# StellaOrg/ImplicitBVH.jl

Measured on AMD Instinct MI355X. Metric: BVH build+traverse throughput, higher is better.
Workload: dtype f32; 1 GPU; 1000000 random BSphere{Float32} leaves per GPU, BBox{Float32} nodes, UInt32 Morton, Int32 index, build + LVT self-traverse + read of the contact count (BASELINE.json configs[1]); leaves_per_gpu=1000000, leaves_total=1000000, contacts_total=1763579, parallelism=single GPU

## Files before the change

implicitbvh.jl_amd/csrc/ibvh_build.hip:

```cpp
#include "ibvh_common.hpp"
#include "ibvh_radix.hpp"
#include "ibvh_msd.hpp"

namespace ibvh {
namespace rsort {
struct FirstPassPlan {
    int tpb, ipt, num_tiles;
    uint32_t *tile_hist;
    uint32_t mask;
    int shift, bits;
};
FirstPassPlan first_pass_plan(int64_t n, int key_bits, int key_bytes, void *scratch);
bool uses_hybrid(int64_t n, int key_bits, int key_bytes);
int sort_pairs(int key_bytes, int key_bits, int64_t n, void *keys, void *vals, void *keys_alt, void *vals_alt,
               bool vals_implicit, int32_t *result_in_alt, void *scratch, size_t scratch_sz, hipStream_t st,
               bool first_hist_done, const RecordArgs *records);
size_t scratch_bytes(int64_t n);
}

namespace build {

constexpr int EXT_TPB = 256;
constexpr int EXT_MAX_BLOCKS = 2048;
constexpr int EXT_FOLD_BLOCKS = 512;

template <class T> IBVH_D T wave_min(T v) {
#pragma unroll
    for (int o = 32; o > 0; o >>= 1) {
        T t = __shfl_xor(v, o, 64);
        v = v < t ? v : t;
    }
    return v;
}
template <class T> IBVH_D T wave_max(T v) {
#pragma unroll
    for (int o = 32; o > 0; o >>= 1) {
        T t = __shfl_xor(v, o, 64);
        v = v > t ? v : t;
    }
    return v;
}

template <class V>
__global__ __launch_bounds__(EXT_TPB) void extrema_partial_kernel(const char *__restrict__ recs, int64_t stride, int64_t n,
                                                                  typename V::elt *__restrict__ partials) {
    using T = typename V::elt;
    T mn[3] = {float_max<T>(), float_max<T>(), float_max<T>()};
    T mx[3] = {float_min_normal<T>(), float_min_normal<T>(), float_min_normal<T>()};
    for (int64_t i = (int64_t)blockIdx.x * EXT_TPB + threadIdx.x; i < n; i += (int64_t)gridDim.x * EXT_TPB) {
        V v = load_vol<V>(recs + i * stride);
        T c[3];
        center(v, c);
#pragma unroll
        for (int k = 0; k < 3; ++k) {
            mn[k] = mn[k] < c[k] ? mn[k] : c[k];
            mx[k] = mx[k] > c[k] ? mx[k] : c[k];
        }
    }
    __shared__ T s[EXT_TPB / 64][6];
    const int lane = threadIdx.x & 63, w = threadIdx.x >> 6;
#pragma unroll
    for (int k = 0; k < 3; ++k) {
        T a = wave_min(mn[k]), b = wave_max(mx[k]);
        if (lane == 0) {
            s[w][k] = a;
            s[w][3 + k] = b;
        }
    }
    __syncthreads();
    if (threadIdx.x < 6) {
        T v = s[0][threadIdx.x];
        for (int i = 1; i < EXT_TPB / 64; ++i) {
            T t = s[i][threadIdx.x];
            v = threadIdx.x < 3 ? (v < t ? v : t) : (v > t ? v : t);
        }
        partials[(int64_t)blockIdx.x * 6 + threadIdx.x] = v;
    }
}

struct SkipsOut {
    TreeDev tree;
    void *skips;
    int index_bytes;
};
IBVH_D void write_skips(const SkipsOut &so) {
    const int64_t level = (int64_t)threadIdx.x + 1;
    if (so.skips == nullptr || level > so.tree.levels) return;
    const int64_t v = level_skips(so.tree.levels, so.tree.virtual_leaves, level);
    if (so.index_bytes == 4) ((int32_t *)so.skips)[level - 1] = (int32_t)v;
    else ((int64_t *)so.skips)[level - 1] = v;
}

template <class T>
__global__ __launch_bounds__(EXT_TPB) void extrema_final_kernel(const T *__restrict__ partials, int nparts, int expand,
                                                                T *__restrict__ out, T *__restrict__ out2, SkipsOut so) {
    write_skips(so);
    T mn[3] = {float_max<T>(), float_max<T>(), float_max<T>()};
    T mx[3] = {float_min_normal<T>(), float_min_normal<T>(), float_min_normal<T>()};
    for (int i = threadIdx.x; i < nparts; i += EXT_TPB) {
#pragma unroll
        for (int k = 0; k < 3; ++k) {
            T a = partials[i * 6 + k], b = partials[i * 6 + 3 + k];
            mn[k] = mn[k] < a ? mn[k] : a;
            mx[k] = mx[k] > b ? mx[k] : b;
        }
    }
    __shared__ T s[EXT_TPB / 64][6];
    const int lane = threadIdx.x & 63, w = threadIdx.x >> 6;
#pragma unroll
    for (int k = 0; k < 3; ++k) {
        T a = wave_min(mn[k]), b = wave_max(mx[k]);
        if (lane == 0) {
            s[w][k] = a;
            s[w][3 + k] = b;
        }
    }
    __syncthreads();
    if (threadIdx.x < 6) {
        T v = s[0][threadIdx.x];
        for (int i = 1; i < EXT_TPB / 64; ++i) {
            T t = s[i][threadIdx.x];
            v = threadIdx.x < 3 ? (v < t ? v : t) : (v > t ? v : t);
        }
        if (expand) {
            const T rp = relative_precision<T>(), fm = float_min_normal<T>();
            T a = rp * ibvh_abs(v);
            v = threadIdx.x < 3 ? (v - a) - fm : (v + a) + fm;
        }
        out[threadIdx.x] = v;
        if (out2) out2[threadIdx.x] = v;
    }
}

template <class T> __global__ void extrema_set_kernel(T *out, T *out2, double a0, double a1, double a2, double b0, double b1, double b2, SkipsOut so) {
    write_skips(so);
    if (threadIdx.x == 0) {
        out[0] = T(a0);
        out[1] = T(a1);
        out[2] = T(a2);
        out[3] = T(b0);
        out[4] = T(b1);
        out[5] = T(b2);
        if (out2)
            for (int k = 0; k < 6; ++k) out2[k] = out[k];
    }
}

template <class V, class K>
__global__ __launch_bounds__(256) void encode_kernel(const char *__restrict__ recs, int64_t stride, int64_t n,
                                                     const typename V::elt *__restrict__ ext, int morton_type,
                                                     K *__restrict__ keys) {
    using T = typename V::elt;
    const T mins[3] = {ext[0], ext[1], ext[2]}, maxs[3] = {ext[3], ext[4], ext[5]};
    for (int64_t i = (int64_t)blockIdx.x * 256 + threadIdx.x; i < n; i += (int64_t)gridDim.x * 256) {
        V v = load_vol<V>(recs + i * stride);
        T c[3];
        center(v, c);
        keys[i] = (K)morton_encode_single(c, mins, maxs, morton_type);
    }
}

template <class T> struct ExtremaFold {
    const T *partials;
    int nparts;
    T *out, *out2;
    SkipsOut so;
};
template <class V, class K>
// ... 24 lines not shown
        for (int k = 0; k < 3; ++k) {
            const T a = wave_min(mn[k]), b = wave_max(mx[k]);
            if (lane == 0) {
                s_fold[w][k] = a;
                s_fold[w][3 + k] = b;
            }
        }
        __syncthreads();
        if (threadIdx.x < 6) {
            T v = s_fold[0][threadIdx.x];
            for (int i = 1; i < (int)(blockDim.x >> 6); ++i) {
                const T t = s_fold[i][threadIdx.x];
                v = threadIdx.x < 3 ? (v < t ? v : t) : (v > t ? v : t);
            }
            const T rp = relative_precision<T>(), fm = float_min_normal<T>();
            const T a = rp * ibvh_abs(v);
            v = threadIdx.x < 3 ? (v - a) - fm : (v + a) + fm;
            s_ext[threadIdx.x] = v;
            if (blockIdx.x == 0) {
                fold.out[threadIdx.x] = v;
                if (fold.out2) fold.out2[threadIdx.x] = v;
            }
        }
    }
    __syncthreads();
    const T *bounds = fold.partials != nullptr ? s_ext : ext;
    const T mins[3] = {bounds[0], bounds[1], bounds[2]}, maxs[3] = {bounds[3], bounds[4], bounds[5]};
    const int64_t base = (int64_t)blockIdx.x * tile_elems;
    for (int j = threadIdx.x; j < tile_elems; j += blockDim.x) {
        const int64_t i = base + j;
        if (i < n) {
            V v = load_vol<V>(recs + i * stride);
            T c[3];
            center(v, c);
            const K k = (K)morton_encode_single(c, mins, maxs, morton_type);
            keys[i] = k;
            atomicAdd(&h[(uint32_t)(k >> shift) & mask], 1u);
        }
    }
    __syncthreads();
    if (tile_major)
        for (int d = threadIdx.x; d <= (int)mask; d += blockDim.x) tile_hist[(int64_t)blockIdx.x * (mask + 1) + d] = h[d];
    else
        for (int d = threadIdx.x; d <= (int)mask; d += blockDim.x) tile_hist[(int64_t)d * num_tiles + blockIdx.x] = h[d];
}

template <class V, class I, class K>
__global__ __launch_bounds__(256) void gather_kernel(const char *__restrict__ src, int64_t src_stride, int src_wrapped,
                                                     LeafLayout lay, const K *__restrict__ keys,
                                                     const uint32_t *__restrict__ perm, int64_t n, char *__restrict__ dst) {
    extern __shared__ __attribute__((aligned(16))) unsigned char g_smem[];
    const int lane = threadIdx.x & 63, wv = threadIdx.x >> 6;
    const int words = lay.stride >> 3;
    uint64_t *stage = (uint64_t *)g_smem + (size_t)wv * 64 * words;
    const int64_t nchunks = ceil_div_dev(n, 256);
    for (int64_t c = blockIdx.x; c < nchunks; c += gridDim.x) {
        const int64_t i = c * 256 + threadIdx.x;
        const int64_t wave_first = c * 256 + wv * 64;
        if (i < n) {
            const uint32_t p = perm[i];
            const char *s = src + (int64_t)p * src_stride;
            V v;
            if (sizeof(V) % 16 == 0 && (src_stride & 15) == 0) v = load_vol16<V>(s);
            else v = load_vol<V>(s);
            I idx = src_wrapped ? load_index<I>(s, lay) : (I)((int64_t)p + 1);
            char *d = (char *)(stage + (size_t)lane * words);
            store_vol(d, v);
            *(I *)(d + lay.index_off) = idx;
            store_morton(d, lay, (uint64_t)keys[i]);
        }
        __builtin_amdgcn_wave_barrier();
        const int64_t wave_n = n - wave_first < 64 ? n - wave_first : 64;
        if (wave_n > 0) {
            uint64_t *out = (uint64_t *)(dst + wave_first * lay.stride);
            const int total = (int)wave_n * words;
            for (int g = lane; g < total; g += 64) out[g] = stage[g];
        }
        __builtin_amdgcn_wave_barrier();
    }
}

constexpr int AGG_TPB = 256;
constexpr int CH_LEVELS = 9;

template <class N>
IBVH_D void fold_up(N *s_nodes, N mine, int64_t level, int64_t nreal, const TreeDev &tree, int64_t built_level, N *__restrict__ nodes) {
    const int t = threadIdx.x;
    int count = AGG_TPB;
#pragma unroll 1
    for (int s = 1; s < CH_LEVELS; ++s) {
        if (level - 1 < built_level) break;
        __syncthreads();
        if (t < count) s_nodes[t] = mine;
        __syncthreads();
        count >>= 1;
        level -= 1;
        const int64_t child_real = nreal;
        nreal = level_num_real(tree.levels, tree.virtual_leaves, level);
        const int64_t i = (int64_t)blockIdx.x * count + t;
        if ((t < count) && (i < nreal)) {
            N a = s_nodes[2 * t];
            if (2 * i + 1 < child_real) mine = merge_to(a, s_nodes[2 * t + 1], (N *)nullptr);
            else mine = a;
            nodes[level_start(tree.levels, tree.virtual_leaves, level) - 1 + i] = mine;
        }
    }
}

template <class L, class N, bool FROM_LEAVES>
__global__ __launch_bounds__(AGG_TPB) void aggregate_kernel(const char *__restrict__ in, int64_t in_stride, int64_t in_level,
                                                            TreeDev tree, int64_t built_level, N *__restrict__ nodes) {
    __shared__ N s_nodes[AGG_TPB];
    const int t = threadIdx.x;
    int64_t level = in_level - 1;
    const int64_t in_real = FROM_LEAVES ? tree.real_leaves : level_num_real(tree.levels, tree.virtual_leaves, in_level);
    const int64_t i = (int64_t)blockIdx.x * AGG_TPB + t;
    const int64_t nreal = level_num_real(tree.levels, tree.virtual_leaves, level);
    N mine;
    if (i < nreal) {
        int64_t l = 2 * i, r = 2 * i + 1;
        if constexpr (FROM_LEAVES) {
            L a = load_vol<L>(in + l * in_stride);
            if (r < in_real) {
                L b = load_vol<L>(in + r * in_stride);
                mine = merge_to(a, b, (N *)nullptr);
            } else {
                mine = convert_to(a, (N *)nullptr);
            }
        } else {
            N a = load_vol<N>(in + l * in_stride);
            if (r < in_real) {
                N b = load_vol<N>(in + r * in_stride);
                mine = merge_to(a, b, (N *)nullptr);
            } else {
                mine = a;
            }
        }
        nodes[level_start(tree.levels, tree.virtual_leaves, level) - 1 + i] = mine;
    }
    fold_up<N>(s_nodes, mine, level, nreal, tree, built_level, nodes);
}

template <class L, class N, class I>
__global__ __launch_bounds__(AGG_TPB) void refit_kernel(char *__restrict__ leaves, LeafLayout lay, const char *__restrict__ volumes,
                                                        int64_t m, uint32_t *flag, TreeDev tree, int64_t built_level,
                                                        N *__restrict__ nodes) {
    __shared__ N s_nodes[AGG_TPB];
    const int64_t i = (int64_t)blockIdx.x * AGG_TPB + threadIdx.x;
    const bool one_leaf = tree.levels == 1;
    const int64_t level = tree.levels - 1;
    const int64_t nreal = one_leaf ? 1 : level_num_real(tree.levels, tree.virtual_leaves, level);
    N mine;
    if (i < nreal) {
        const bool has_b = !one_leaf && 2 * i + 1 < tree.real_leaves;
        char *ra = leaves + 2 * i * lay.stride, *rb = ra + lay.stride;
        const I ia = load_index<I>(ra, lay), ib = has_b ? load_index<I>(rb, lay) : I(1);
        const bool oka = ia >= 1 && (int64_t)ia <= m, okb = ib >= 1 && (int64_t)ib <= m;
        const char *sa = oka ? volumes + ((int64_t)ia - 1) * (int64_t)sizeof(L) : ra;
        const char *sb = okb ? volumes + ((int64_t)ib - 1) * (int64_t)sizeof(L) : rb;
        L a, b;
        if constexpr (sizeof(L) % 16 == 0) {
            a = oka && ((uintptr_t)volumes & 15) == 0 ? load_vol16<L>(sa) : load_vol<L>(sa);
            if (has_b) b = okb && ((uintptr_t)volumes & 15) == 0 ? load_vol16<L>(sb) : load_vol<L>(sb);
        } else {
            a = load_vol<L>(sa);
            if (has_b) b = load_vol<L>(sb);
        }
        if (oka) store_vol(ra, a);
        if (has_b && okb) store_vol(rb, b);
        if (flag && !(oka && okb)) *flag = 1u;
        if (one_leaf) return;
        mine = has_b ? merge_to(a, b, (N *)nullptr) : convert_to(a, (N *)nullptr);
        nodes[level_start(tree.levels, tree.virtual_leaves, level) - 1 + i] = mine;
    }
    if (one_leaf) return;
    fold_up<N>(s_nodes, mine, level, nreal, tree, built_level, nodes);
}

constexpr int AGG_TOP_TPB = 1024, AGG_TOP_MAX = 4096, AGG_TOP_LDS_BYTES = 128 * 1024;
template <class N, bool IN_LDS>
__global__ __launch_bounds__(AGG_TOP_TPB) void aggregate_top_kernel(TreeDev tree, int64_t in_level, int64_t built_level, N *nodes) {
    if constexpr (IN_LDS) {
        extern __shared__ __attribute__((aligned(16))) unsigned char top_smem[];
        N *s = (N *)top_smem;
        int64_t have = level_num_real(tree.levels, tree.virtual_leaves, in_level);
        {
            const N *in = nodes + (level_start(tree.levels, tree.virtual_leaves, in_level) - 1);
            for (int64_t i = threadIdx.x; i < have; i += AGG_TOP_TPB) s[i] = load_vol<N>(in + i);
        }
        __syncthreads();
        for (int64_t level = in_level - 1; level >= built_level && level >= 1; --level) {
            const int64_t nreal = level_num_real(tree.levels, tree.virtual_leaves, level);
            N *out = nodes + (level_start(tree.levels, tree.virtual_leaves, level) - 1);
            N mine[2];
#pragma unroll
            for (int k = 0; k < 2; ++k) {
                const int64_t i = threadIdx.x + (int64_t)k * AGG_TOP_TPB;
                if (i < nreal) mine[k] = (2 * i + 1 < have) ? merge_to(s[2 * i], s[2 * i + 1], (N *)nullptr) : s[2 * i];
            }
            __syncthreads();
#pragma unroll
            for (int k = 0; k < 2; ++k) {
                const int64_t i = threadIdx.x + (int64_t)k * AGG_TOP_TPB;
                if (i < nreal) {
                    s[i] = mine[k];
                    store_vol(out + i, mine[k]);
                }
            }
            __syncthreads();
            have = nreal;
        }
        return;
    }
    for (int64_t level = in_level - 1; level >= built_level && level >= 1; --level) {
        const int64_t nreal = level_num_real(tree.levels, tree.virtual_leaves, level);
        const int64_t child_real = level_num_real(tree.levels, tree.virtual_leaves, level + 1);
        const N *in = nodes + (level_start(tree.levels, tree.virtual_leaves, level + 1) - 1);
        N *out = nodes + (level_start(tree.levels, tree.virtual_leaves, level) - 1);
        for (int64_t i = threadIdx.x; i < nreal; i += AGG_TOP_TPB) {
            const N a = load_vol<N>(in + 2 * i);
            if (2 * i + 1 < child_real) store_vol(out + i, merge_to(a, load_vol<N>(in + 2 * i + 1), (N *)nullptr));
            else store_vol(out + i, a);
        }
        __threadfence_block();
        __syncthreads();
    }
}

struct RefitGather {
    LeafLayout lay;
    int index_type;
    const void *volumes;
    int64_t m;
    uint32_t *flag;
};

template <class L, class N>
int aggregate(const char *leaves, int64_t leaf_stride, const ibvh_tree &tree, int64_t built_level, N *nodes, hipStream_t st,
              const RefitGather *gather = nullptr) {
    if (tree.real_nodes < 2 && !gather) return IBVH_OK;
    TreeDev td{tree.levels, tree.real_leaves, tree.virtual_leaves};
    int64_t in_level = tree.levels;
    {
        int64_t nreal = tree.levels > 1 ? level_num_real(tree.levels, tree.virtual_leaves, in_level - 1) : 1;
        int64_t eff_built = built_level > tree.levels - 1 ? tree.levels - 1 : built_level;
        if (gather) {
            int e = dispatch_index(gather->index_type, [&](auto it) -> int {
                using I = typename decltype(it)::type;
                IBVH_LAUNCH((refit_kernel<L, N, I>), dim3((unsigned)ceil_div(nreal, AGG_TPB)), dim3(AGG_TPB), 0, st,
                            (char *)leaves, gather->lay, (const char *)gather->volumes, gather->m, gather->flag, td, eff_built, nodes);
                return IBVH_OK;
            });
            if (e) return e;
        } else {
            IBVH_LAUNCH((aggregate_kernel<L, N, true>), dim3((unsigned)ceil_div(nreal, AGG_TPB)), dim3(AGG_TPB), 0, st,
                               leaves, leaf_stride, in_level, td, eff_built, nodes);
        }
        IBVH_LAUNCH_CHECK();
        if (tree.real_nodes < 2) return IBVH_OK;
        in_level = in_level - CH_LEVELS;
    }
    while (in_level - 1 >= built_level && in_level - 1 >= 1) {
        if (level_num_real(tree.levels, tree.virtual_leaves, in_level) <= AGG_TOP_MAX) {
            const size_t top_bytes = (size_t)level_num_real(tree.levels, tree.virtual_leaves, in_level) * sizeof(N);
            if (top_bytes <= (size_t)AGG_TOP_LDS_BYTES) {
                IBVH_HIP_CHECK(hipFuncSetAttribute((const void *)aggregate_top_kernel<N, true>, hipFuncAttributeMaxDynamicSharedMemorySize, AGG_TOP_LDS_BYTES));
                IBVH_LAUNCH((aggregate_top_kernel<N, true>), dim3(1), dim3(AGG_TOP_TPB), top_bytes, st, td, in_level, built_level, nodes);
            } else {
                IBVH_LAUNCH((aggregate_top_kernel<N, false>), dim3(1), dim3(AGG_TOP_TPB), 0, st, td, in_level, built_level, nodes);
            }
            IBVH_LAUNCH_CHECK();
            break;
        }
        int64_t nreal = level_num_real(tree.levels, tree.virtual_leaves, in_level - 1);
        const char *in = (const char *)(nodes + (level_start(tree.levels, tree.virtual_leaves, in_level) - 1));
        IBVH_LAUNCH((aggregate_kernel<L, N, false>), dim3((unsigned)ceil_div(nreal, AGG_TPB)), dim3(AGG_TPB), 0, st,
                           in, (int64_t)sizeof(N), in_level, td, built_level, nodes);
        IBVH_LAUNCH_CHECK();
        in_level -= CH_LEVELS;
    }
    return IBVH_OK;
}

template <class I> __global__ void skips_kernel(TreeDev tree, I *skips) {
    int64_t level = threadIdx.x + 1;
    if (level <= tree.levels) skips[level - 1] = (I)level_skips(tree.levels, tree.virtual_leaves, level);
}

inline int grid_for(int64_t n, int tpb, int max_blocks) {
    int64_t b = ceil_div(n, tpb);
    return (int)(b < 1 ? 1 : (b > max_blocks ? max_blocks : b));
}

struct Scratch {
    char *partials;
    char *extrema;
    char *keys, *keys_alt;
    char *vals, *vals_alt;
    char *records;
    char *records2;
    char *sort;
    size_t total;
};
inline int morton_key_bits(int morton_type);
inline Scratch carve(char *base, int64_t n, int key_bytes, int64_t leaf_bytes, int morton_type) {
    Scratch s;
    size_t off = 0;
    auto take = [&](size_t bytes) {
        char *p = base ? base + off : nullptr;
        off += (size_t)align_up((int64_t)bytes, 256);
        return p;
    };
    s.partials = take((size_t)EXT_MAX_BLOCKS * 6 * 8);
    s.extrema = take(64);
    s.keys = take((size_t)n * key_bytes);
    s.keys_alt = take((size_t)n * key_bytes);
    s.vals = take((size_t)n * 4);
    s.vals_alt = take((size_t)n * 4);
    s.records = take((size_t)n * leaf_bytes);
    s.records2 = take((size_t)n * leaf_bytes);
    const size_t a = rsort::scratch_bytes(n), b = msd::scratch_bytes(n, morton_key_bits(morton_type), key_bytes, (int)leaf_bytes);
    s.sort = take(a > b ? a : b);
    s.total = off;
    return s;
}

template <class V> int extrema_partials(const char *recs, int64_t stride, int64_t n, char *partials, hipStream_t st, int *nparts) {
    using T = typename V::elt;
    const int blocks = grid_for(n, EXT_TPB * 4, EXT_FOLD_BLOCKS);
    IBVH_LAUNCH((extrema_partial_kernel<V>), dim3(blocks), dim3(EXT_TPB), 0, st, recs, stride, n, (T *)partials);
    *nparts = blocks;
    return IBVH_OK;
}
template <class V>
int extrema(const char *recs, int64_t stride, int64_t n, int expand, typename V::elt *out, char *partials, hipStream_t st,
            typename V::elt *out2 = nullptr, SkipsOut so = SkipsOut{TreeDev{0, 0, 0}, nullptr, 4}) {
    using T = typename V::elt;
    int blocks = grid_for(n, EXT_TPB * 4, EXT_MAX_BLOCKS);
    IBVH_LAUNCH((extrema_partial_kernel<V>), dim3(blocks), dim3(EXT_TPB), 0, st, recs, stride, n, (T *)partials);
    IBVH_LAUNCH((extrema_final_kernel<T>), dim3(1), dim3(EXT_TPB), 0, st, (const T *)partials, blocks, expand, out, out2, so);
    IBVH_LAUNCH_CHECK();
    return IBVH_OK;
}

template <class V>
int encode(const char *recs, int64_t stride, int64_t n, const typename V::elt *ext, int morton_type, void *keys, hipStream_t st) {
    int blocks = grid_for(n, 256, 256 * 16);
    if (morton_type == IBVH_U64)
        IBVH_LAUNCH((encode_kernel<V, uint64_t>), dim3(blocks), dim3(256), 0, st, recs, stride, n, ext, morton_type,
                           (uint64_t *)keys);
    else
        IBVH_LAUNCH((encode_kernel<V, uint32_t>), dim3(blocks), dim3(256), 0, st, recs, stride, n, ext, morton_type,
                           (uint32_t *)keys);
    IBVH_LAUNCH_CHECK();
    return IBVH_OK;
}

inline int morton_key_bits(int morton_type) { return morton_type == IBVH_U16 ? 15 : (morton_type == IBVH_U32 ? 30 : 63); }

}
}

using namespace ibvh;
using namespace ibvh::build;

extern "C" {

ibvh_status ibvh_build_scratch_bytes(const ibvh_types *types, int64_t n, size_t *bytes_out) {
    if (!types || !bytes_out) return IBVH_ERR_INVALID_ARG;
    ibvh_layout lay;
    if (!layout_of(*types, lay)) return IBVH_ERR_UNSUPPORTED;
    if (n < 1) return IBVH_ERR_DOMAIN;
    int kb = types->morton_type == IBVH_U64 ? 8 : 4;
    *bytes_out = carve(nullptr, n, kb, lay.leaf_bytes, types->morton_type).total;
    return IBVH_OK;
}

ibvh_status ibvh_extrema(const ibvh_types *types, const void *records, int32_t wrapped, int64_t n, int32_t expand,
                         void *extrema_out, void *scratch, size_t scratch_bytes, void *stream) {
    if (!types || !records || !extrema_out || !scratch) return IBVH_ERR_INVALID_ARG;
    if (n < 1) return IBVH_ERR_DOMAIN;
    if (scratch_bytes < (size_t)EXT_MAX_BLOCKS * 6 * 8) return IBVH_ERR_SCRATCH;
    ibvh_layout lay;
    if (!layout_of(*types, lay)) return IBVH_ERR_UNSUPPORTED;
    int64_t stride = wrapped ? lay.leaf_bytes : lay.volume_bytes;
    return (ibvh_status)dispatch_volume(types->leaf_kind, types->leaf_float, [&](auto lt) -> int {
        using V = typename decltype(lt)::type;
        return extrema<V>((const char *)records, stride, n, expand, (typename V::elt *)extrema_out, (char *)scratch,
                          (hipStream_t)stream);
    });
}

ibvh_status ibvh_morton_keys(const ibvh_types *types, const void *records, int32_t wrapped, int64_t n, const void *ext,
                             void *keys_out, void *stream) {
    if (!types || !records || !ext || !keys_out) return IBVH_ERR_INVALID_ARG;
    if (n < 1) return IBVH_ERR_DOMAIN;
    ibvh_layout lay;
    if (!layout_of(*types, lay)) return IBVH_ERR_UNSUPPORTED;
    int64_t stride = wrapped ? lay.leaf_bytes : lay.volume_bytes;
    return (ibvh_status)dispatch_volume(types->leaf_kind, types->leaf_float, [&](auto lt) -> int {
        using V = typename decltype(lt)::type;
        return encode<V>((const char *)records, stride, n, (const typename V::elt *)ext, types->morton_type, keys_out,
                         (hipStream_t)stream);
    });
}

ibvh_status ibvh_aggregate(const ibvh_types *types, const ibvh_tree *tree, int64_t built_level, const void *leaves,
                           void *nodes, void *stream) {
    if (!types || !tree || !leaves) return IBVH_ERR_INVALID_ARG;
    if (built_level < 1 || built_level > tree->levels) return IBVH_ERR_INVALID_ARG;
    ibvh_layout lay;
    if (!layout_of(*types, lay)) return IBVH_ERR_UNSUPPORTED;
    if (tree->real_nodes >= 2 && !nodes) return IBVH_ERR_INVALID_ARG;
    return (ibvh_status)dispatch_leaf_node(*types, [&](auto lt, auto nt) -> int {
        using L = typename decltype(lt)::type;
        using N = typename decltype(nt)::type;
        return aggregate<L, N>((const char *)leaves, lay.leaf_bytes, *tree, built_level, (N *)nodes, (hipStream_t)stream);
    });
}

ibvh_status ibvh_refit(const ibvh_bvh *bvh, const void *volumes, int64_t num_volumes, void *flag, void *stream) {
    if (!bvh || !bvh->leaves) return IBVH_ERR_INVALID_ARG;
    const ibvh_tree &tree = bvh->tree;
    if (tree.real_leaves < 1 || tree.levels < 1) return IBVH_ERR_INVALID_ARG;
    if (bvh->built_level < 1 || bvh->built_level > tree.levels) return IBVH_ERR_INVALID_ARG;
    if (tree.real_nodes >= 2 && !bvh->nodes) return IBVH_ERR_INVALID_ARG;
    if (volumes && (num_volumes < 0 || ((uintptr_t)volumes & 7) != 0)) return IBVH_ERR_INVALID_ARG;
    ibvh_layout lay;
    LeafLayout dlay;
    if (!layout_of(bvh->types, lay, &dlay)) return IBVH_ERR_UNSUPPORTED;
    const RefitGather g{dlay, bvh->types.index_type, volumes, num_volumes, (uint32_t *)flag};
    return (ibvh_status)dispatch_leaf_node(bvh->types, [&](auto lt, auto nt) -> int {
        using L = typename decltype(lt)::type;
        using N = typename decltype(nt)::type;
        return aggregate<L, N>((const char *)bvh->leaves, lay.leaf_bytes, tree, bvh->built_level, (N *)bvh->nodes,
                               (hipStream_t)stream, volumes ? &g : nullptr);
    });
}

ibvh_status ibvh_build(const ibvh_build_desc *desc, const void *volumes, void *leaves, void *nodes, void *skips,
                       void *extrema_out, void *scratch, size_t scratch_bytes, void *stream) {
    if (!desc || !leaves || !skips || !scratch) return IBVH_ERR_INVALID_ARG;
    const ibvh_types &ty = desc->types;
    ibvh_layout lay;
    LeafLayout dlay;
    if (!layout_of(ty, lay, &dlay)) return IBVH_ERR_UNSUPPORTED;
    ibvh_tree tree;
    if (ibvh_status e = ibvh_tree_shape(desc->n, &tree)) return e;
    if (desc->n >= (int64_t(1) << 32)) return IBVH_ERR_INVALID_ARG;
    if (ty.index_type == IBVH_I32 && tree.real_nodes > INT32_MAX) return IBVH_ERR_OVERFLOW;
    if (desc->built_level < 1 || desc->built_level > tree.levels) return IBVH_ERR_INVALID_ARG;
    if (!desc->already_wrapped && !volumes) return IBVH_ERR_INVALID_ARG;
    if (tree.real_nodes >= 2 && !nodes) return IBVH_ERR_INVALID_ARG;
    const int64_t n = desc->n;
    const int key_bytes = ty.morton_type == IBVH_U64 ? 8 : 4;
    const bool wrapped = desc->already_wrapped != 0;
    Scratch sc = carve((char *)scratch, n, key_bytes, lay.leaf_bytes, ty.morton_type);
    if (scratch_bytes < sc.total) return IBVH_ERR_SCRATCH;
    hipStream_t st = (hipStream_t)stream;

    const bool out_of_place = wrapped && volumes != nullptr;
    const char *src = wrapped ? (out_of_place ? (const char *)volumes : (const char *)leaves) : (const char *)volumes;
    const int64_t src_stride = wrapped ? lay.leaf_bytes : lay.volume_bytes;

    int rc = dispatch_leaf_node(ty, [&](auto lt, auto nt) -> int {
        using L = typename decltype(lt)::type;
        using N = typename decltype(nt)::type;
        using T = typename L::elt;
        T *ext = (T *)sc.extrema;
        TreeDev td{tree.levels, tree.real_leaves, tree.virtual_leaves};
        const SkipsOut so{td, skips, ty.index_type == IBVH_I32 ? 4 : 8};
        ExtremaFold<T> fold{nullptr, 0, ext, (T *)extrema_out, so};
        const bool fold_in_encode = n <= (int64_t)1 << 21;
        if (desc->compute_extrema && fold_in_encode) {
            int nparts = 0;
            if (int e = extrema_partials<L>(src, src_stride, n, sc.partials, st, &nparts)) return e;
            fold.partials = (const T *)sc.partials;
            fold.nparts = nparts;
        } else if (desc->compute_extrema) {
            if (int e = extrema<L>(src, src_stride, n, 1, ext, sc.partials, st, (T *)extrema_out, so)) return e;
        } else {
            IBVH_LAUNCH((extrema_set_kernel<T>), dim3(1), dim3(64), 0, st, ext, (T *)extrema_out, desc->mins[0], desc->mins[1],
                               desc->mins[2], desc->maxs[0], desc->maxs[1], desc->maxs[2], so);
        }
        const int key_bits = morton_key_bits(ty.morton_type);
        const msd::Plan mp = msd::make_plan(n, key_bits, key_bytes, (int)lay.leaf_bytes, sc.sort);
        rsort::FirstPassPlan plan;
        if (mp.bits) plan = rsort::FirstPassPlan{mp.ptpb, mp.pipt, mp.num_tiles, mp.tb.tile_hist, (1u << mp.bits) - 1u, mp.shift, mp.bits};
        else plan = rsort::first_pass_plan(n, key_bits, key_bytes, sc.sort);
        if (key_bytes == 8)
            IBVH_LAUNCH((encode_hist_kernel<L, uint64_t>), dim3(plan.num_tiles), dim3(plan.tpb), ((size_t)plan.mask + 1) * 4, st,
                        src, src_stride, n, ext, ty.morton_type, (uint64_t *)sc.keys, plan.tpb * plan.ipt, plan.shift, plan.mask,
                        plan.tile_hist, plan.num_tiles, mp.bits ? 1 : 0, fold);
        else
            IBVH_LAUNCH((encode_hist_kernel<L, uint32_t>), dim3(plan.num_tiles), dim3(plan.tpb), ((size_t)plan.mask + 1) * 4, st,
                        src, src_stride, n, ext, ty.morton_type, (uint32_t *)sc.keys, plan.tpb * plan.ipt, plan.shift, plan.mask,
                        plan.tile_hist, plan.num_tiles, mp.bits ? 1 : 0, fold);
        IBVH_LAUNCH_CHECK();
        if (mp.bits) {
            rsort::RecordArgs ra{src, sc.records, src_stride, wrapped ? 1 : 0, (int32_t)(lay.volume_bytes / 8),
                                 ty.index_type == IBVH_I32 ? 4 : 8, dlay};
            if (int e = msd::sort_records(mp, key_bytes, key_bits, sc.keys, n, ra, sc.records2, (char *)leaves, sc.keys_alt, (uint32_t *)sc.vals_alt, sc.keys,
                                          (uint32_t *)sc.vals, desc->sort_levels, desc->sort_equalize != 0, desc->skew_flag, st))
                return e;
            return aggregate<L, N>((const char *)leaves, lay.leaf_bytes, tree, desc->built_level, (N *)nodes, st);
        }
        if (desc->skew_flag) IBVH_HIP_CHECK(hipMemsetAsync(desc->skew_flag, 0, 4, st));
        char *dst = (wrapped && !out_of_place) ? sc.records : (char *)leaves;
        const bool fuse_records = rsort::uses_hybrid(n, key_bits, key_bytes) || n < (int64_t(1) << 22);
        rsort::RecordArgs ra{src, dst, src_stride, wrapped ? 1 : 0, (int32_t)(lay.volume_bytes / 8),
                             ty.index_type == IBVH_I32 ? 4 : 8, dlay};
        int32_t in_alt = 0;
        if (int e = rsort::sort_pairs(key_bytes, key_bits, n, sc.keys, sc.vals, sc.keys_alt, sc.vals_alt, true, &in_alt,
                                      sc.sort, rsort::scratch_bytes(n), st, true, fuse_records ? &ra : nullptr))
            return e;
        if (!fuse_records) {
            const void *skeys = in_alt ? sc.keys_alt : sc.keys;
            const uint32_t *sperm = (const uint32_t *)(in_alt ? sc.vals_alt : sc.vals);
            int gblocks = grid_for(n, 256, 256 * 16);
            auto launch_gather = [&](auto it) -> int {
                using I = typename decltype(it)::type;
                const size_t gsm = (size_t)256 * lay.leaf_bytes;
                if (key_bytes == 8)
                    IBVH_LAUNCH((gather_kernel<L, I, uint64_t>), dim3(gblocks), dim3(256), gsm, st, src, src_stride,
                                wrapped ? 1 : 0, dlay, (const uint64_t *)skeys, sperm, n, dst);
                else
                    IBVH_LAUNCH((gather_kernel<L, I, uint32_t>), dim3(gblocks), dim3(256), gsm, st, src, src_stride,
                                wrapped ? 1 : 0, dlay, (const uint32_t *)skeys, sperm, n, dst);
                return IBVH_OK;
            };
            if (int e = dispatch_index(ty.index_type, launch_gather)) return e;
            IBVH_LAUNCH_CHECK();
        }
        if (wrapped && !out_of_place)
            IBVH_HIP_CHECK(hipMemcpyAsync(leaves, sc.records, (size_t)n * lay.leaf_bytes, hipMemcpyDeviceToDevice, st));
        return aggregate<L, N>((const char *)leaves, lay.leaf_bytes, tree, desc->built_level, (N *)nodes, st);
    });
    return (ibvh_status)rc;
}

}
```

implicitbvh.jl_amd/csrc/ibvh_common.hpp:

```cpp
#pragma once
#include <hip/hip_runtime.h>
#include <stdint.h>

#include "../../include/ibvh.h"

#define IBVH_HD __host__ __device__ __forceinline__
#define IBVH_D __device__ __forceinline__

namespace ibvh {

template <class T> struct BSphere {
    using elt = T;
    static constexpr int kind = IBVH_BSPHERE;
    T x[3];
    T r;
};
template <class T> struct BBox {
    using elt = T;
    static constexpr int kind = IBVH_BBOX;
    T lo[3];
    T up[3];
};
template <class I> struct IndexPair {
    I a, b;
// ... 358 lines not shown
inline bool layout_of(const ibvh_types &t, ibvh_layout &out, LeafLayout *dev = nullptr) {
    if (!combo_ok(t)) return false;
    int64_t fl = t.leaf_float == IBVH_F32 ? 4 : 8, fn = t.node_float == IBVH_F32 ? 4 : 8;
    int64_t vb = (t.leaf_kind == IBVH_BSPHERE ? 4 : 6) * fl;
    int64_t nb = (t.node_kind == IBVH_BSPHERE ? 4 : 6) * fn;
    int64_t ib = t.index_type == IBVH_I32 ? 4 : 8;
    int64_t mb = t.morton_type == IBVH_U16 ? 2 : (t.morton_type == IBVH_U32 ? 4 : 8);
    int64_t io = align_up(vb, ib);
    int64_t mo = align_up(io + ib, mb);
    int64_t al = fl > ib ? fl : ib;
    al = al > mb ? al : mb;
    out.volume_bytes = vb;
    out.node_bytes = nb;
    out.index_off = io;
    out.morton_off = mo;
    out.leaf_bytes = align_up(mo + mb, al);
    out.pair_bytes = 2 * ib;
    if (dev) *dev = {(int32_t)out.leaf_bytes, (int32_t)io, (int32_t)mo, (int32_t)mb};
    return true;
}

template <class F> int dispatch_volume(int kind, int flt, F &&f) {
    if (kind == IBVH_BSPHERE && flt == IBVH_F32) return f(Tag<BSphere<float>>{});
    if (kind == IBVH_BBOX && flt == IBVH_F32) return f(Tag<BBox<float>>{});
#ifndef IBVH_ONLY_BENCH_TYPES
    if (kind == IBVH_BSPHERE && flt == IBVH_F64) return f(Tag<BSphere<double>>{});
    if (kind == IBVH_BBOX && flt == IBVH_F64) return f(Tag<BBox<double>>{});
#endif
    return IBVH_ERR_UNSUPPORTED;
}
template <class F> int dispatch_leaf_node(const ibvh_types &t, F &&f) {
    if (!combo_ok(t)) return IBVH_ERR_UNSUPPORTED;
    return dispatch_volume(t.leaf_kind, t.leaf_float, [&](auto lt) -> int {
        using L = typename decltype(lt)::type;
        return dispatch_volume(t.node_kind, t.node_float, [&](auto nt) -> int {
            using N = typename decltype(nt)::type;
            constexpr bool ok = !(N::kind == IBVH_BSPHERE && L::kind != IBVH_BSPHERE);
            if constexpr (ok) return f(lt, nt);
            else return (int)IBVH_ERR_UNSUPPORTED;
        });
    });
}
template <class F> int dispatch_index(int index_type, F &&f) {
    if (index_type == IBVH_I32) return f(Tag<int32_t>{});
#ifndef IBVH_ONLY_BENCH_TYPES
    if (index_type == IBVH_I64) return f(Tag<int64_t>{});
#endif
    return IBVH_ERR_UNSUPPORTED;
}

#define IBVH_HIP_CHECK(expr)                                  \
    do {                                                      \
        hipError_t _e = (expr);                               \
        if (_e != hipSuccess) return (int)IBVH_ERR_HIP;       \
    } while (0)
#define IBVH_LAUNCH_CHECK()                                   \
    do {                                                      \
        if (hipGetLastError() != hipSuccess) return (int)IBVH_ERR_HIP; \
    } while (0)

inline int64_t ceil_div(int64_t a, int64_t b) { return (a + b - 1) / b; }
IBVH_HD int64_t ceil_div_dev(int64_t a, int64_t b) { return (a + b - 1) / b; }

struct Tuning {
    int ray_block = 0;
    int lvt_wide = 0;
    int msd_rescue = 1;
    int lvt_blocks = 1;
    int lvt_block_shift = 0;
    int lvt_blocks_paired_below = -1;
    int lvt_blocks_min_items = 0;
    int lvt_xcd = 64;
    int sort_lsd = 0;
    int sort_msd_avg = 1536;
    int msd = 1;
    int msd_avg = 1024;
    int lvt_scan_fused = 1;
    int msd_equalize = 0;
    int bfs_wg_per_cu = 4;
    int rays_binned = 1;
    int rays_subtree_depth = 0;
    int rays_tail = 8;
    int rays_items_per_ray = 0;
};
extern Tuning g_tuning;

namespace prof {
extern bool enabled;
void begin(const char *name, hipStream_t st);
void end(hipStream_t st);
}
#define IBVH_LAUNCH(kernel, grid, block, smem, st, ...)                          \
    do {                                                                         \
        if (::ibvh::prof::enabled) ::ibvh::prof::begin(#kernel, st);             \
        hipLaunchKernelGGL(kernel, grid, block, smem, st, __VA_ARGS__);          \
        if (::ibvh::prof::enabled) ::ibvh::prof::end(st);                        \
    } while (0)

IBVH_D int xcd_remap(int b, int nwg) {
    const int q = nwg >> 3, r = nwg & 7;
    const int xcd = b & 7, k = b >> 3;
    return (xcd < r ? xcd * (q + 1) : r * (q + 1) + (xcd - r) * q) + k;
}

IBVH_D int xcd_run_remap(int b, int nwg, int run) {
    if ((run & (run - 1)) == 0) {
        const int sh = __builtin_ctz((unsigned)run);
        const int full = (nwg >> (sh + 3)) << (sh + 3);
        if (b >= full) return b;
        const int xcd = b & 7, k = b >> 3;
        return ((((k >> sh) << 3) + xcd) << sh) + (k & (run - 1));
    }
    const int period = 8 * run;
    const int full = (nwg / period) * period;
    if (b >= full) return b;
    const int xcd = b & 7, k = b >> 3;
    return ((k / run) * 8 + xcd) * run + (k % run);
}

IBVH_D int lane_id() { return (int)__builtin_amdgcn_mbcnt_hi(~0u, __builtin_amdgcn_mbcnt_lo(~0u, 0u)); }

}
```

implicitbvh.jl_amd/csrc/ibvh_core.hip:

```cpp
#include <cmath>

#include "ibvh_common.hpp"

#include <mutex>
#include <string>
#include <vector>

using namespace ibvh;

namespace ibvh {
namespace prof {
bool enabled = false;
struct Rec {
    std::string name;
    hipEvent_t a, b;
};
static std::vector<Rec> recs;
static std::vector<hipEvent_t> pool;
static std::mutex mu;
static thread_local size_t last = 0;
static hipEvent_t take() {
    hipEvent_t e;
    if (!pool.empty()) {
        e = pool.back();
        pool.pop_back();
        return e;
    }
    (void)hipEventCreate(&e);
    return e;
}
void begin(const char *name, hipStream_t st) {
    std::lock_guard<std::mutex> g(mu);
    Rec r{name, take(), take()};
    (void)hipEventRecord(r.a, st);
    recs.push_back(r);
    last = recs.size() - 1;
}
void end(hipStream_t st) {
    std::lock_guard<std::mutex> g(mu);
    if (last < recs.size()) (void)hipEventRecord(recs[last].b, st);
}
static void reset() {
    std::lock_guard<std::mutex> g(mu);
    for (auto &r : recs) {
        pool.push_back(r.a);
        pool.push_back(r.b);
    }
    recs.clear();
}
}
}

namespace ibvh {
Tuning g_tuning;
}
namespace {
struct Knob {
    const char *name;
    int Tuning::*field;
};
const Knob kKnobs[] = {
    {"ray_block", &Tuning::ray_block},   {"lvt_wide", &Tuning::lvt_wide},     {"lvt_xcd", &Tuning::lvt_xcd},
    {"sort_lsd", &Tuning::sort_lsd},     {"sort_msd_avg", &Tuning::sort_msd_avg}, {"msd", &Tuning::msd},
    {"msd_avg", &Tuning::msd_avg},       {"msd_equalize", &Tuning::msd_equalize}, {"msd_rescue", &Tuning::msd_rescue}, {"lvt_scan_fused", &Tuning::lvt_scan_fused}, {"bfs_wg_per_cu", &Tuning::bfs_wg_per_cu},
    {"lvt_blocks", &Tuning::lvt_blocks}, {"lvt_block_shift", &Tuning::lvt_block_shift}, {"lvt_blocks_min_items", &Tuning::lvt_blocks_min_items}, {"lvt_blocks_paired_below", &Tuning::lvt_blocks_paired_below},
    {"rays_binned", &Tuning::rays_binned}, {"rays_subtree_depth", &Tuning::rays_subtree_depth},
    {"rays_items_per_ray", &Tuning::rays_items_per_ray}, {"rays_tail", &Tuning::rays_tail},
};
inline int64_t ilog2_down(int64_t n) { return 63 - __builtin_clzll((unsigned long long)n); }
}

extern "C" {

ibvh_status ibvh_tree_shape(int64_t num_leaves, ibvh_tree *out) {
    if (!out) return IBVH_ERR_INVALID_ARG;
    if (num_leaves < 1) return IBVH_ERR_DOMAIN;
    if (num_leaves > (int64_t(1) << 60)) return IBVH_ERR_INVALID_ARG;
    int64_t lr = num_leaves;
    int64_t fl = ilog2_down(lr);
    int64_t levels = ((lr & (lr - 1)) == 0 ? fl : fl + 1) + 1;
    int64_t lv = (int64_t(1) << (levels - 1)) - lr;
    out->levels = levels;
    out->real_leaves = lr;
    out->real_nodes = 2 * lr - 1 + popc64(lv);
    out->virtual_leaves = lv;
    out->virtual_nodes = 2 * lv - popc64(lv);
    return IBVH_OK;
}

ibvh_status ibvh_compute_skips(const ibvh_tree *tree, int64_t *skips_out) {
    if (!tree || !skips_out) return IBVH_ERR_INVALID_ARG;
    for (int64_t level = 1; level <= tree->levels; ++level)
        skips_out[level - 1] = level_skips(tree->levels, tree->virtual_leaves, level);
    return IBVH_OK;
}

ibvh_status ibvh_memory_index(const ibvh_tree *tree, int64_t implicit_index, int64_t *out) {
    if (!tree || !out) return IBVH_ERR_INVALID_ARG;
    if (!(1 <= implicit_index && implicit_index <= (int64_t(1) << tree->levels) - 1)) return IBVH_ERR_INVALID_ARG;
    int64_t level = ilog2_down(implicit_index) + 1;
    *out = implicit_index - level_skips(tree->levels, tree->virtual_leaves, level);
    return IBVH_OK;
}

ibvh_status ibvh_level_indices(const ibvh_tree *tree, int64_t level, int64_t *start, int64_t *stop) {
    if (!tree || !start || !stop) return IBVH_ERR_INVALID_ARG;
    if (!(1 <= level && level <= tree->levels)) return IBVH_ERR_INVALID_ARG;
    *start = level_start(tree->levels, tree->virtual_leaves, level);
    *stop = *start + level_num_real(tree->levels, tree->virtual_leaves, level) - 1;
    return IBVH_OK;
}

ibvh_status ibvh_isvirtual(const ibvh_tree *tree, int64_t implicit_index, int32_t *out) {
    if (!tree || !out) return IBVH_ERR_INVALID_ARG;
    if (!(1 <= implicit_index && implicit_index <= (int64_t(1) << tree->levels) - 1)) return IBVH_ERR_INVALID_ARG;
    int64_t level = ilog2_down(implicit_index) + 1;
    int64_t first = int64_t(1) << (level - 1);
    *out = (implicit_index - first + 1 > level_num_real(tree->levels, tree->virtual_leaves, level)) ? 1 : 0;
    return IBVH_OK;
}

ibvh_status ibvh_compute_build_level(const ibvh_tree *tree, double frac, int64_t *out) {
    if (!tree || !out) return IBVH_ERR_INVALID_ARG;
    if (!(0.0 <= frac && frac <= 1.0)) return IBVH_ERR_INVALID_ARG;
    double x = double(tree->levels) + double(1 - tree->levels) * frac;
    *out = (int64_t)std::nearbyint(x);
    return IBVH_OK;
}

ibvh_status ibvh_layout_of(const ibvh_types *types, ibvh_layout *out) {
    if (!types || !out) return IBVH_ERR_INVALID_ARG;
    return layout_of(*types, *out) ? IBVH_OK : IBVH_ERR_UNSUPPORTED;
}

ibvh_status ibvh_profile_enable(int32_t on) {
    prof::reset();
    prof::enabled = on != 0;
    return IBVH_OK;
}
ibvh_status ibvh_profile_count(int64_t *count_out) {
    if (!count_out) return IBVH_ERR_INVALID_ARG;
    *count_out = (int64_t)prof::recs.size();
    return IBVH_OK;
}
ibvh_status ibvh_profile_get(int64_t i, const char **name_out, float *ms_out) {
    if (!name_out || !ms_out || i < 0 || i >= (int64_t)prof::recs.size()) return IBVH_ERR_INVALID_ARG;
    auto &r = prof::recs[(size_t)i];
    if (hipEventSynchronize(r.b) != hipSuccess) return IBVH_ERR_HIP;
    if (hipEventElapsedTime(ms_out, r.a, r.b) != hipSuccess) return IBVH_ERR_HIP;
    *name_out = r.name.c_str();
// ... 42 lines not shown
```

Before: 4492 Mleaves/s.

## Fuse top-of-tree aggregation into leaf aggregate kernel via last-block arrival counters

The leaf-level aggregate kernel now publishes each block's top node with agent-scope stores and increments hierarchical arrival counters. The last block to arrive then folds the remaining upper levels itself, replacing the separate top-aggregation launch(es). The counters are zeroed inside the extrema final kernel, so no extra memset is needed. This removes kernel launch and dependency overhead at the cost of a serial tail done by a single block, and the result depends on memory-ordering correctness of relaxed atomics plus an s_waitcnt.

New measurement: 4492 Mleaves/s (median of 3 runs). Within noise of the previous version (+0.0%).

```diff
diff --git a/implicitbvh.jl_amd/csrc/ibvh_build.hip b/implicitbvh.jl_amd/csrc/ibvh_build.hip
--- a/implicitbvh.jl_amd/csrc/ibvh_build.hip
+++ b/implicitbvh.jl_amd/csrc/ibvh_build.hip
@@ -78,12 +78,17 @@
     }
 }
 
+constexpr int AGG_ARRIVE_GROUPS = 16;
+constexpr int AGG_ARRIVE_WORDS = AGG_ARRIVE_GROUPS + 1;
+constexpr int AGG_ARRIVE_STRIDE = 32;
 struct SkipsOut {
     TreeDev tree;
     void *skips;
     int index_bytes;
+    uint32_t *arrive;
 };
 IBVH_D void write_skips(const SkipsOut &so) {
+    if (so.arrive != nullptr && threadIdx.x < AGG_ARRIVE_WORDS) so.arrive[threadIdx.x * AGG_ARRIVE_STRIDE] = 0u;
     const int64_t level = (int64_t)threadIdx.x + 1;
     if (so.skips == nullptr || level > so.tree.levels) return;
     const int64_t v = level_skips(so.tree.levels, so.tree.virtual_leaves, level);
@@ -274,9 +279,10 @@
 
 constexpr int AGG_TPB = 256;
 constexpr int CH_LEVELS = 9;
+constexpr int AGG_TOP_MAX = 4096;
 
 template <class N>
-IBVH_D void fold_up(N *s_nodes, N mine, int64_t level, int64_t nreal, const TreeDev &tree, int64_t built_level, N *__restrict__ nodes) {
+IBVH_D void fold_up(N *s_nodes, N &mine, int64_t level, int64_t nreal, const TreeDev &tree, int64_t built_level, N *__restrict__ nodes) {
     const int t = threadIdx.x;
     int count = AGG_TPB;
 #pragma unroll 1
@@ -299,9 +305,90 @@
     }
 }
 
-template <class L, class N, bool FROM_LEAVES>
+template <class N> IBVH_D void store_vol_agent(N *p, const N &v) {
+    static_assert(sizeof(N) % 8 == 0, "volumes are multiples of 8 bytes");
+    uint64_t w[sizeof(N) / 8];
+    __builtin_memcpy(w, &v, sizeof(N));
+#pragma unroll
+    for (int k = 0; k < (int)(sizeof(N) / 8); ++k) __hip_atomic_store((uint64_t *)p + k, w[k], __ATOMIC_RELAXED, __HIP_MEMORY_SCOPE_AGENT);
+}
+template <class N> IBVH_D N load_vol_agent(const N *p) {
+    static_assert(sizeof(N) % 8 == 0, "volumes are multiples of 8 bytes");
+    uint64_t w[sizeof(N) / 8];
+#pragma unroll
+    for (int k = 0; k < (int)(sizeof(N) / 8); ++k) w[k] = __hip_atomic_load((uint64_t *)const_cast<N *>(p) + k, __ATOMIC_RELAXED, __HIP_MEMORY_SCOPE_AGENT);
+    N v;
+    __builtin_memcpy(&v, w, sizeof(N));
+    return v;
+}
+
+template <class N> constexpr bool AGG_FOLD_TOP_OK = sizeof(N) <= 32;
+template <class N>
+IBVH_D void fold_top(N *s_nodes, const TreeDev &tree, int64_t in_level, int64_t built_level, N *nodes) {
+    static_assert(16 * AGG_TPB >= AGG_TOP_MAX, "sixteen inputs a thread");
+    constexpr int RUN = sizeof(N) <= 24 ? 4 : 2, RUN_LEVELS = RUN == 4 ? 2 : 1, MAX_ACC = 4 - RUN_LEVELS;
+    const int t = threadIdx.x;
+    const int64_t stop = built_level > 1 ? built_level : 1;
+    const int64_t have = level_num_real(tree.levels, tree.virtual_leaves, in_level);
+    const N *in = nodes + (level_start(tree.levels, tree.virtual_leaves, in_level) - 1);
+    int shift = RUN_LEVELS;
+    while (((int64_t)AGG_TPB << shift) < have) ++shift;
+    auto parent = [&](const N &a, const N &b, int64_t i, int64_t level) -> N {
+        const int64_t child_real = level_num_real(tree.levels, tree.virtual_leaves, level + 1);
+        const N m = (2 * i + 1 < child_real) ? merge_to(a, b, (N *)nullptr) : a;
+        if (i < level_num_real(tree.levels, tree.virtual_leaves, level) && level >= stop)
+            store_vol(nodes + (level_start(tree.levels, tree.virtual_leaves, level) - 1) + i, m);
+        return m;
+    };
+    N acc[MAX_ACC + 1];
+#pragma unroll
+    for (int h = 0; h < 16 / RUN; ++h) {
+        if (RUN * h >= (1 << shift)) break;
+        const int64_t first = ((int64_t)t << shift) + RUN * h;
+        N v[RUN];
+#pragma unroll
+        for (int k = 0; k < RUN; ++k)
+            if (first + k < have) v[k] = load_vol_agent(in + first + k);
+#pragma unroll
+        for (int s = 1; s <= RUN_LEVELS; ++s)
+#pragma unroll
+            for (int k = 0; k < (RUN >> s); ++k) v[k] = parent(v[2 * k], v[2 * k + 1], (first >> s) + k, in_level - s);
+        N c = v[0];
+        int b = 0;
+#pragma unroll
+        for (; (h >> b) & 1; ++b) c = parent(acc[b], c, first >> (RUN_LEVELS + b + 1), in_level - (RUN_LEVELS + b + 1));
+        acc[b] = c;
+    }
+    int64_t level = in_level - shift;
+    if (level < stop) return;
+    int64_t nreal = level_num_real(tree.levels, tree.virtual_leaves, level);
+    N mine = acc[0];
+#pragma unroll
+    for (int b = 1; b <= MAX_ACC; ++b)
+        if (shift - RUN_LEVELS == b) mine = acc[b];
+    int count = AGG_TPB;
+#pragma unroll 1
+    while (level - 1 >= stop) {
+        __syncthreads();
+        if (t < count) s_nodes[t] = mine;
+        __syncthreads();
+        count >>= 1;
+        level -= 1;
+        const int64_t child_real = nreal;
+        nreal = level_num_real(tree.levels, tree.virtual_leaves, level);
+        if ((t < count) && (t < nreal)) {
+            N a = s_nodes[2 * t];
+            if (2 * (int64_t)t + 1 < child_real) mine = merge_to(a, s_nodes[2 * t + 1], (N *)nullptr);
+            else mine = a;
+            store_vol(nodes + (level_start(tree.levels, tree.virtual_leaves, level) - 1) + t, mine);
+        }
+    }
+}
+
+template <class L, class N, bool FROM_LEAVES, bool FOLD_TOP = false>
 __global__ __launch_bounds__(AGG_TPB) void aggregate_kernel(const char *__restrict__ in, int64_t in_stride, int64_t in_level,
-                                                            TreeDev tree, int64_t built_level, N *__restrict__ nodes) {
+                                                            TreeDev tree, int64_t built_level, N *__restrict__ nodes,
+                                                            uint32_t *arrive) {
     __shared__ N s_nodes[AGG_TPB];
     const int t = threadIdx.x;
     int64_t level = in_level - 1;
@@ -331,6 +418,25 @@
         nodes[level_start(tree.levels, tree.virtual_leaves, level) - 1 + i] = mine;
     }
     fold_up<N>(s_nodes, mine, level, nreal, tree, built_level, nodes);
+    if constexpr (FOLD_TOP) {
+        const int64_t top_level = in_level - CH_LEVELS;
+        uint32_t *s_last = (uint32_t *)s_nodes;
+        __syncthreads();
+        if (t == 0) {
+            store_vol_agent(nodes + (level_start(tree.levels, tree.virtual_leaves, top_level) - 1) + blockIdx.x, mine);
+            asm volatile("s_waitcnt vmcnt(0)" ::: "memory");
+            const uint32_t g = blockIdx.x % AGG_ARRIVE_GROUPS;
+            const uint32_t members = (gridDim.x + AGG_ARRIVE_GROUPS - 1 - g) / AGG_ARRIVE_GROUPS;
+            const uint32_t groups = gridDim.x < (uint32_t)AGG_ARRIVE_GROUPS ? gridDim.x : (uint32_t)AGG_ARRIVE_GROUPS;
+            uint32_t last = 0;
+            if (__hip_atomic_fetch_add(arrive + g * AGG_ARRIVE_STRIDE, 1u, __ATOMIC_RELAXED, __HIP_MEMORY_SCOPE_AGENT) == members - 1)
+                last = __hip_atomic_fetch_add(arrive + AGG_ARRIVE_GROUPS * AGG_ARRIVE_STRIDE, 1u, __ATOMIC_RELAXED, __HIP_MEMORY_SCOPE_AGENT) == groups - 1;
+            *s_last = last;
+        }
+        __syncthreads();
+        if (__builtin_amdgcn_readfirstlane((int)*s_last) == 0) return;
+        fold_top<N>(s_nodes, tree, top_level, built_level, nodes);
+    }
 }
 
 template <class L, class N, class I>
@@ -369,7 +475,7 @@
     fold_up<N>(s_nodes, mine, level, nreal, tree, built_level, nodes);
 }
 
-constexpr int AGG_TOP_TPB = 1024, AGG_TOP_MAX = 4096, AGG_TOP_LDS_BYTES = 128 * 1024;
+constexpr int AGG_TOP_TPB = 1024, AGG_TOP_LDS_BYTES = 128 * 1024;
 template <class N, bool IN_LDS>
 __global__ __launch_bounds__(AGG_TOP_TPB) void aggregate_top_kernel(TreeDev tree, int64_t in_level, int64_t built_level, N *nodes) {
     if constexpr (IN_LDS) {
@@ -429,9 +535,12 @@
 
 template <class L, class N>
 int aggregate(const char *leaves, int64_t leaf_stride, const ibvh_tree &tree, int64_t built_level, N *nodes, hipStream_t st,
-              const RefitGather *gather = nullptr) {
+              const RefitGather *gather = nullptr, uint32_t *arrive = nullptr) {
     if (tree.real_nodes < 2 && !gather) return IBVH_OK;
     TreeDev td{tree.levels, tree.real_leaves, tree.virtual_leaves};
+    const int64_t top_level = tree.levels - CH_LEVELS;
+    const bool fold_top_here = AGG_FOLD_TOP_OK<N> && arrive != nullptr && !gather && g_tuning.agg_fold_top != 0 && top_level - 1 >= built_level &&
+                               top_level - 1 >= 1 && level_num_real(tree.levels, tree.virtual_leaves, top_level) <= AGG_TOP_MAX;
     int64_t in_level = tree.levels;
     {
         int64_t nreal = tree.levels > 1 ? level_num_real(tree.levels, tree.virtual_leaves, in_level - 1) : 1;
@@ -444,9 +553,16 @@
                 return IBVH_OK;
             });
             if (e) return e;
+        } else if (fold_top_here) {
+            if constexpr (AGG_FOLD_TOP_OK<N>) {
+                IBVH_LAUNCH((aggregate_kernel<L, N, true, true>), dim3((unsigned)ceil_div(nreal, AGG_TPB)), dim3(AGG_TPB), 0, st,
+                                   leaves, leaf_stride, in_level, td, eff_built, nodes, arrive);
+                IBVH_LAUNCH_CHECK();
+                return IBVH_OK;
+            }
         } else {
             IBVH_LAUNCH((aggregate_kernel<L, N, true>), dim3((unsigned)ceil_div(nreal, AGG_TPB)), dim3(AGG_TPB), 0, st,
-                               leaves, leaf_stride, in_level, td, eff_built, nodes);
+                               leaves, leaf_stride, in_level, td, eff_built, nodes, (uint32_t *)nullptr);
         }
         IBVH_LAUNCH_CHECK();
         if (tree.real_nodes < 2) return IBVH_OK;
@@ -467,7 +583,7 @@
         int64_t nreal = level_num_real(tree.levels, tree.virtual_leaves, in_level - 1);
         const char *in = (const char *)(nodes + (level_start(tree.levels, tree.virtual_leaves, in_level) - 1));
         IBVH_LAUNCH((aggregate_kernel<L, N, false>), dim3((unsigned)ceil_div(nreal, AGG_TPB)), dim3(AGG_TPB), 0, st,
-                           in, (int64_t)sizeof(N), in_level, td, built_level, nodes);
+                           in, (int64_t)sizeof(N), in_level, td, built_level, nodes, (uint32_t *)nullptr);
         IBVH_LAUNCH_CHECK();
         in_level -= CH_LEVELS;
     }
@@ -487,6 +603,7 @@
 struct Scratch {
     char *partials;
     char *extrema;
+    char *agg_arrive;
     char *keys, *keys_alt;
     char *vals, *vals_alt;
     char *records;
@@ -505,6 +622,7 @@
     };
     s.partials = take((size_t)EXT_MAX_BLOCKS * 6 * 8);
     s.extrema = take(64);
+    s.agg_arrive = take((size_t)AGG_ARRIVE_WORDS * AGG_ARRIVE_STRIDE * 4);
     s.keys = take((size_t)n * key_bytes);
     s.keys_alt = take((size_t)n * key_bytes);
     s.vals = take((size_t)n * 4);
@@ -661,7 +779,7 @@
         using T = typename L::elt;
         T *ext = (T *)sc.extrema;
         TreeDev td{tree.levels, tree.real_leaves, tree.virtual_leaves};
-        const SkipsOut so{td, skips, ty.index_type == IBVH_I32 ? 4 : 8};
+        const SkipsOut so{td, skips, ty.index_type == IBVH_I32 ? 4 : 8, (uint32_t *)sc.agg_arrive};
         ExtremaFold<T> fold{nullptr, 0, ext, (T *)extrema_out, so};
         const bool fold_in_encode = n <= (int64_t)1 << 21;
         if (desc->compute_extrema && fold_in_encode) {
@@ -695,7 +813,7 @@
             if (int e = msd::sort_records(mp, key_bytes, key_bits, sc.keys, n, ra, sc.records2, (char *)leaves, sc.keys_alt, (uint32_t *)sc.vals_alt, sc.keys,
                                           (uint32_t *)sc.vals, desc->sort_levels, desc->sort_equalize != 0, desc->skew_flag, st))
                 return e;
-            return aggregate<L, N>((const char *)leaves, lay.leaf_bytes, tree, desc->built_level, (N *)nodes, st);
+            return aggregate<L, N>((const char *)leaves, lay.leaf_bytes, tree, desc->built_level, (N *)nodes, st, nullptr, (uint32_t *)sc.agg_arrive);
         }
         if (desc->skew_flag) IBVH_HIP_CHECK(hipMemsetAsync(desc->skew_flag, 0, 4, st));
         char *dst = (wrapped && !out_of_place) ? sc.records : (char *)leaves;
@@ -726,7 +844,7 @@
         }
         if (wrapped && !out_of_place)
             IBVH_HIP_CHECK(hipMemcpyAsync(leaves, sc.records, (size_t)n * lay.leaf_bytes, hipMemcpyDeviceToDevice, st));
-        return aggregate<L, N>((const char *)leaves, lay.leaf_bytes, tree, desc->built_level, (N *)nodes, st);
+        return aggregate<L, N>((const char *)leaves, lay.leaf_bytes, tree, desc->built_level, (N *)nodes, st, nullptr, (uint32_t *)sc.agg_arrive);
     });
     return (ibvh_status)rc;
 }
diff --git a/implicitbvh.jl_amd/csrc/ibvh_common.hpp b/implicitbvh.jl_amd/csrc/ibvh_common.hpp
--- a/implicitbvh.jl_amd/csrc/ibvh_common.hpp
+++ b/implicitbvh.jl_amd/csrc/ibvh_common.hpp
@@ -464,6 +464,7 @@
     int rays_subtree_depth = 0;
     int rays_tail = 8;
     int rays_items_per_ray = 0;
+    int agg_fold_top = 1;
 };
 extern Tuning g_tuning;
 
diff --git a/implicitbvh.jl_amd/csrc/ibvh_core.hip b/implicitbvh.jl_amd/csrc/ibvh_core.hip
--- a/implicitbvh.jl_amd/csrc/ibvh_core.hip
+++ b/implicitbvh.jl_amd/csrc/ibvh_core.hip
@@ -66,6 +66,7 @@
     {"lvt_blocks", &Tuning::lvt_blocks}, {"lvt_block_shift", &Tuning::lvt_block_shift}, {"lvt_blocks_min_items", &Tuning::lvt_blocks_min_items}, {"lvt_blocks_paired_below", &Tuning::lvt_blocks_paired_below},
     {"rays_binned", &Tuning::rays_binned}, {"rays_subtree_depth", &Tuning::rays_subtree_depth},
     {"rays_items_per_ray", &Tuning::rays_items_per_ray}, {"rays_tail", &Tuning::rays_tail},
+    {"agg_fold_top", &Tuning::agg_fold_top},
 };
 inline int64_t ilog2_down(int64_t n) { return 63 - __builtin_clzll((unsigned long long)n); }
 }
```
